# daniabib/ComfyUI_ProPainter_Nodes

Hardware: NVIDIA H100
Metric: inpainted frames/sec at 640x360, 80-frame subvideo (higher is better)
Workload: dtype f16

## Files before the change

### comfyui_propainter_nodes_b200/csrc/capi.cu

```cuda
#include <math.h>
#include <string.h>

#include <thread>
#include <vector>

#include "../../include/propainter_b200.h"
#include "engine.cuh"

struct DeviceGuard {
  int prev = -1;
  bool changed = false, ok = true;
  explicit DeviceGuard(int dev) {
    if (cudaGetDevice(&prev) != cudaSuccess) prev = -1;
    if (prev != dev) {
      ok = cudaSetDevice(dev) == cudaSuccess;
      changed = ok;
    }
  }
  ~DeviceGuard() {
    if (changed && prev >= 0) cudaSetDevice(prev);
  }
};

#define PP_HANDLE(h)                                     \
// ... 409 lines not shown
    a.n++; a.ms += ms; a.rows += r.rows; a.flops += r.flops; a.bytes += r.bytes;
  }
  size_t off = 0;
  buf[0] = 0;
  for (auto& kv : agg) {
    char line[512];
    int n = snprintf(line, sizeof(line), "%s\t%lld\t%.6f\t%.0f\t%.0f\t%.0f\n", kv.first.c_str(), kv.second.n,
                     kv.second.ms, kv.second.rows, kv.second.flops, kv.second.bytes);
    if (off + n + 1 > cap) { pp_set_error("pp_profile_dump: buffer too small"); return PP_ERR_ARG; }
    memcpy(buf + off, line, n + 1);
    off += n;
  }
  return PP_OK;
}

int pp_op_conv(pp_handle h, const char* name, const void* x_f16, int N, int H, int W, int stride, int pad, int dil,
               int replicate, int act, float slope, const void* residual_f16, void* out_f16, void* stream) {
  PP_HANDLE(h);
  const PPPackedConv* w = nullptr;
  PP_TRY(pp_get_conv(e, name, &w));
  PPConvCall c(e, name, N, H, W);
  c.in(static_cast<const __half*>(x_f16), w->cin_g * w->groups, 0, w->cin_g, w->groups > 1 ? w->cin_g : 0)
      .geom(stride, stride, pad, pad, dil, dil, replicate)
      .out(static_cast<__half*>(out_f16), w->cout_g * w->groups, 0, w->groups > 1 ? w->cout_g : 0)
      .act(act, slope);
  if (residual_f16 != nullptr) c.residual(static_cast<const __half*>(residual_f16), w->cout_g * w->groups, 0);
  return c.run(as_stream(stream));
}

int pp_op_corr_lookup(pp_handle h, const void* l0, const void* l1, const void* l2, const void* l3,
                      const float* coords, void* out_f16, long long nq, int h8, int w8, void* stream) {
  PP_HANDLE(h);
  e.launches++;
  return pp_k_corr_lookup(static_cast<const __half*>(l0), static_cast<const __half*>(l1),
                          static_cast<const __half*>(l2), static_cast<const __half*>(l3), coords,
                          static_cast<__half*>(out_f16), 328, nq, h8, w8, as_stream(stream));
}

int pp_op_conv_tf32(pp_handle h, const char* name, const float* x0, int x0_C, int x0_co, int x0_ch, const float* x1,
                    int x1_C, int x1_co, int x1_ch, int N, int H, int W, int sh, int sw, int ph, int pw, int dh, int dw,
                    int replicate, int epi, int act, float slope, float scale, int act2, const float* aux0, int aux0_C, int aux0_co, float* aux1,
// ... 117 lines not shown
```

### comfyui_propainter_nodes_b200/csrc/conv_epilogue.cuh

```cuda
#pragma once
#include "conv_igemm.cuh"
#include "wgmma_ops.cuh"

namespace ppconv {

template <int ACT, bool ACC = false, int N>
__device__ __forceinline__ void act16_t(float (&v)[N], float slope) {
#pragma unroll
  for (int i = 0; i < N; ++i) {
    if (ACT == PP_ACT_RELU) v[i] = fmaxf(v[i], 0.f);
    else if (ACT == PP_ACT_LRELU) v[i] = v[i] > 0.f ? v[i] : v[i] * slope;
    else if (ACT == PP_ACT_SIGMOID) v[i] = ppx::sigmoidf_(v[i]);
    else if (ACT == PP_ACT_TANH) v[i] = ACC ? ppx::tanh_acc(v[i]) : tanhf(v[i]);
    else if (ACT == PP_ACT_GELU) v[i] = ppx::gelu_erf(v[i]);
  }
}
template <bool ACC = false, int N>
__device__ __forceinline__ void act16(float (&v)[N], int act, float slope) {
  switch (act) {
    case PP_ACT_RELU: act16_t<PP_ACT_RELU, ACC>(v, slope); break;
    case PP_ACT_LRELU: act16_t<PP_ACT_LRELU, ACC>(v, slope); break;
    case PP_ACT_SIGMOID: act16_t<PP_ACT_SIGMOID, ACC>(v, slope); break;
    case PP_ACT_TANH: act16_t<PP_ACT_TANH, ACC>(v, slope); break;
    case PP_ACT_GELU: act16_t<PP_ACT_GELU, ACC>(v, slope); break;
// ... 232 lines not shown
#pragma unroll
    for (int i = 0; i < 16; i += 4) {
      const float4 v = *reinterpret_cast<const float4*>(src + i);
      acc[i] = v.x; acc[i + 1] = v.y; acc[i + 2] = v.z; acc[i + 3] = v.w;
    }
    conv_epilogue16_split(p, acc, mrow, g, ng0, p.vec_ok != 0);
  } else {
    uint32_t raw[16];
#pragma unroll
    for (int i = 0; i < 16; i += 4) {
      const float4 v = *reinterpret_cast<const float4*>(src + i);
      raw[i] = __float_as_uint(v.x); raw[i + 1] = __float_as_uint(v.y);
      raw[i + 2] = __float_as_uint(v.z); raw[i + 3] = __float_as_uint(v.w);
    }
    conv_epilogue16(p, raw, mrow, g, ng0, EPI >= 0 ? EPI : p.epi, p.vec_ok != 0);
  }
}

template <int V>
struct IntC { static constexpr int value = V; };
template <int MAX_N, class F>
__device__ __forceinline__ void with_tile_width(int bn, F&& f) {
  switch (bn) {
    case 16: f(IntC<16>{}); break;
    case 32: f(IntC<32>{}); break;
    case 48: f(IntC<48>{}); break;
    case 64: f(IntC<64>{}); break;
    case 80: f(IntC<80>{}); break;
    case 96: f(IntC<96>{}); break;
    case 112: f(IntC<112>{}); break;
// ... 22 lines not shown
```

### comfyui_propainter_nodes_b200/csrc/conv_halo.cu

```cuda
#include <cuda.h>
#include <stdlib.h>
#include <string.h>

#include <memory>

#include "conv_epilogue.cuh"
#include "conv_igemm.cuh"
#include "dcn_sample.cuh"

namespace {

constexpr int NUM_THREADS = 384;
constexpr int NUM_EPI_THREADS = 256;
constexpr int WARP_A = 8, WARP_B = 9;
constexpr int MAX_SA = 4, MAX_SB = 8;
constexpr int SMEM_BUDGET = 186 * 1024;

struct HaloParams {
  PPConvParams c;
  CUtensorMap tmap[PP_MAX_SEGS];
  int MT;
  int BW, BH;
  int tiles_x, tiles_y, n_tiles;
  int a_stage_bytes, b_stage_bytes, SA, SB;
// ... 16 lines not shown
  t.ty = r % h.tiles_y; r /= h.tiles_y;
  t.img = r % h.n_img;
  t.g = r / h.n_img;
  return t;
}

__host__ __device__ inline int halo_total_tiles(const HaloParams& h) {
  return h.n_tiles * h.tiles_x * h.tiles_y * h.n_img * h.c.groups;
}

struct Ring {
  int s;
  uint32_t ph;
};

struct HaloSmem {
  uint8_t* a;
  uint8_t* b;
  int SA, SB, a_stage_bytes, b_stage_bytes;
  uint64_t *a_full, *a_empty, *b_full, *b_empty;
  uint64_t* spare;
  float* acc_stg;
  int bytes;
};

__host__ __device__ inline HaloSmem halo_smem(uint8_t* base, int SA, int a_stage_bytes, int SB, int b_stage_bytes) {
  const int b_off = SA * a_stage_bytes, bar_off = b_off + SB * b_stage_bytes, acc_off = bar_off + 1024;
  HaloSmem m;
  m.SA = SA; m.SB = SB; m.a_stage_bytes = a_stage_bytes; m.b_stage_bytes = b_stage_bytes;
  m.a = base;
  m.b = base + b_off;
  m.a_full = reinterpret_cast<uint64_t*>(base + bar_off);
  m.a_empty = m.a_full + MAX_SA;
  m.b_full = m.a_empty + MAX_SA;
  m.b_empty = m.b_full + MAX_SB;
  m.spare = m.b_empty + MAX_SB;
  m.acc_stg = reinterpret_cast<float*>(base + acc_off);
  m.bytes = 1024 + acc_off + 2 * ppconv::STG_BYTES;
  return m;
}

__host__ __device__ constexpr int halo_max_tps(int bn) { return 128 / bn > 1 ? 128 / bn : 1; }

template <int BN, int MB, bool TF32>
__device__ __forceinline__ void halo_tap(float (&acc)[MB][BN / 2], uint64_t (&adesc)[MB], uint64_t& bdesc, uint32_t& accum,
                                         int& kx, int kw, uint32_t step_x, uint32_t step_row, uint32_t tap16) {
#pragma unroll
  for (int k = 0; k < 4; ++k)
#pragma unroll
    for (int b = 0; b < MB; ++b) {
      if constexpr (TF32) ppx::wgmma_tf32<BN>(acc[b], adesc[b] + 2 * k, bdesc + 2 * k, (accum | k) != 0 ? 1u : 0u);
      else ppx::wgmma_f16<BN>(acc[b], adesc[b] + 2 * k, bdesc + 2 * k, (accum | k) != 0 ? 1u : 0u);
    }
  accum = 1u;
// ... 9 lines not shown
                                               uint32_t& accum, int& kx, int kw, uint32_t step_x, uint32_t step_row,
                                               uint32_t tap16) {
  using namespace ppx;
  if constexpr (NT > 1) {
    if (tn < NT) {
      halo_tap_group<BN, MB, NT - 1, TF32>(tn, acc, adesc, bdesc, accum, kx, kw, step_x, step_row, tap16);
      return;
    }
  }
  wgmma_fence();
#pragma unroll
  for (int tt = 0; tt < NT; ++tt) halo_tap<BN, MB, TF32>(acc, adesc, bdesc, accum, kx, kw, step_x, step_row, tap16);
  wgmma_commit();
}

template <int BN, int MB, int NT, bool TF32 = false, bool PROG = false>
__device__ __forceinline__ void halo_tile(const HaloParams& h, int tile, const HaloSmem& m, Ring& ra, Ring& rb, float* stg,
                                          int wg, int t128) {
  using namespace ppx;
  const PPConvParams& p = h.c;
  const int taps = p.kh * p.kw;
  const TileCoord t = decode_tile(h, tile);
  const int n0 = t.n_idx * p.BN;
  const int bnt = min(p.BN, p.Cout_g_pad - n0);
  const uint32_t sbo = h.flat ? 1024u : (uint32_t)h.BW * 128;
  const uint32_t step_x = (uint32_t)p.dw * 8;
  const uint32_t step_row = (uint32_t)(p.dh * h.BW - (p.kw - 1) * p.dw) * 8;
  const uint32_t tap16 = (uint32_t)p.BN * 8;
  const int kw = p.kw;
  uint32_t aoff[MB];
#pragma unroll
  for (int b = 0; b < MB; ++b) aoff[b] = MB == 2 ? wg * h.sub_bytes + b * 8 * sbo : wg * 8 * sbo;
  float acc[MB][BN / 2];
// ... 6 lines not shown
    for (int b = 0; b < MB; ++b) adesc[b] = gmma_desc_sw128_kmajor(smem_u32(m.a + ra.s * m.a_stage_bytes) + aoff[b], sbo);
    int kx = 0;
    for (int tap0 = 0; tap0 < taps; tap0 += h.tps) {
      mbar_wait(&m.b_full[rb.s], rb.ph);
      const uint64_t bdesc = gmma_desc_sw128_kmajor(smem_u32(m.b + rb.s * m.b_stage_bytes));
      halo_tap_group<BN, MB, NT, TF32>(min(h.tps, taps - tap0), acc, adesc, bdesc, accum, kx, kw, step_x, step_row, tap16);
      wgmma_wait<1>();
      if (pend_b >= 0) mbar_arrive(&m.b_empty[pend_b]);
      if (pend_a >= 0) mbar_arrive(&m.a_empty[pend_a]);
      pend_b = rb.s;
      pend_a = tap0 + h.tps >= taps ? ra.s : -1;
      if (++rb.s == m.SB) { rb.s = 0; rb.ph ^= 1; }
    }
    if (++ra.s == m.SA) { ra.s = 0; ra.ph ^= 1; }
  }
  wgmma_wait<0>();
#pragma unroll
  for (int b = 0; b < MB; ++b) wgmma_fence_acc(acc[b]);
  if (pend_b >= 0) mbar_arrive(&m.b_empty[pend_b]);
  if (pend_a >= 0) mbar_arrive(&m.a_empty[pend_a]);

  const bool skip = (h.debug & 1) != 0;
#pragma unroll
  for (int b = 0; b < MB; ++b) {
    const int sub = MB == 2 ? wg : 0, rbase = MB == 2 ? 64 * b : 64 * wg;
    ppconv::drain_acc<BN>(acc[b], stg, t128, 4 + wg, [&](const float* src, int r64, int cc) {
      const int r = rbase + r64;
      bool mvalid;
      long long mrow;
      if (h.flat) {
        mrow = ((long long)t.tx * h.MT + sub) * 128 + r;
        mvalid = mrow < p.M_total;
      } else {
        const int oy = t.ty * 16 + (r >> 3), ox = t.tx * (8 * h.MT) + 8 * sub + (r & 7);
        mvalid = oy < p.OH && ox < p.OW;
        mrow = ((long long)t.img * p.OH + oy) * p.OW + ox;
      }
      if (!mvalid || skip || cc >= bnt || n0 + cc >= p.Cout_g) return;
      ppconv::epilogue_from_stage<TF32, PROG ? PP_EPI_STD : -1>(p, src, mrow, t.g, n0 + cc);
    });
  }
}

template <class F>
__device__ __forceinline__ void with_tile_shape(int mt, int bn, F&& f) {
  if (mt == 2) ppconv::with_tile_width<128>(bn, [&](auto n) { f(n, ppconv::IntC<2>{}); });
  else ppconv::with_tile_width<256>(bn, [&](auto n) { f(n, ppconv::IntC<1>{}); });
}

__device__ __forceinline__ void halo_smem_init_barriers(const HaloSmem& m) {
  using namespace ppx;
  for (int s = 0; s < m.SA; ++s) { mbar_init(&m.a_full[s], 1); mbar_init(&m.a_empty[s], NUM_EPI_THREADS); }
  for (int s = 0; s < m.SB; ++s) { mbar_init(&m.b_full[s], 1); mbar_init(&m.b_empty[s], NUM_EPI_THREADS); }
  mbar_fence_init();
}

__device__ __forceinline__ void halo_produce_patches(const HaloParams& h, const HaloSmem& m, Ring& r) {
  using namespace ppx;
  const PPConvParams& p = h.c;
  const int total_tiles = halo_total_tiles(h);
  const uint32_t bytes = (uint32_t)(h.BW * h.BH * 128);
  for (int tile = blockIdx.x; tile < total_tiles; tile += gridDim.x) {
// ... 39 lines not shown

template <bool TF32>
__device__ __forceinline__ void halo_body(const HaloParams& h) {
  using namespace ppx;
  const HaloSmem m = halo_smem(dyn_smem_1024(), h.SA, h.a_stage_bytes, h.SB, h.b_stage_bytes);
  const int tid = threadIdx.x, warp = tid >> 5;
  if (tid == 0) halo_smem_init_barriers(m);
  __syncthreads();
  asm volatile("griddepcontrol.wait;" ::: "memory");
  asm volatile("griddepcontrol.launch_dependents;" ::: "memory");

  if (warp < 8) setmaxnreg_inc<232>();
  else setmaxnreg_dec<40>();
  if (warp < 8) {
    const int wg = tid >> 7, t128 = tid & 127;
    float* stg = m.acc_stg + wg * (ppconv::STG_BYTES / 4);
    Ring ra = {0, 0}, rb = {0, 0};
    const int total_tiles = halo_total_tiles(h);
    with_tile_shape(h.MT, h.c.BN, [&](auto bn, auto mb) {
      constexpr int BN = decltype(bn)::value;
      for (int tile = blockIdx.x; tile < total_tiles; tile += gridDim.x)
        halo_tile<BN, decltype(mb)::value, halo_max_tps(BN), TF32>(h, tile, m, ra, rb, stg, wg, t128);
    });
  } else if (warp == WARP_A) {
    if (elect_one()) {
      Ring r = {0, 0};
      halo_produce_patches(h, m, r);
    }
  } else if (warp == WARP_B) {
    if (elect_one()) {
      Ring r = {0, 0};
      halo_produce_weights(h, m, r);
    }
  }
}

__global__ void __launch_bounds__(NUM_THREADS, 1) conv_halo_kernel(const __grid_constant__ HaloParams h) {
  halo_body<false>(h);
}

__global__ void __launch_bounds__(NUM_THREADS, 1) conv_halo_tf32_kernel(const __grid_constant__ HaloParams h) {
  halo_body<true>(h);
}

constexpr int PROG_MAX_LAYERS = 10;
enum { PROG_CONV = 0, PROG_DCN = 1 };

constexpr int PROG_WIDTHS[] = {32, 64, 224};

template <class F>
__device__ __forceinline__ void with_prog_width(int bn, F&& f) {
  static_assert(sizeof(PROG_WIDTHS) == 3 * sizeof(int), "with_prog_width: one case per PROG_WIDTHS entry");
  switch (bn) {
    case PROG_WIDTHS[0]: f(ppconv::IntC<PROG_WIDTHS[0]>{}); break;
    case PROG_WIDTHS[1]: f(ppconv::IntC<PROG_WIDTHS[1]>{}); break;
    case PROG_WIDTHS[2]: f(ppconv::IntC<PROG_WIDTHS[2]>{}); break;
    default: __trap();
  }
}

struct ProgParams {
  int n_layers;
  int SA, SB, a_stage_bytes, b_stage_bytes;
// ... 28 lines not shown

  const int tid = threadIdx.x, warp = tid >> 5;
  const unsigned int G = gridDim.x;
  if (tid == 0) {
    mbar_init(layer_go, 1);
    halo_smem_init_barriers(m);
  }
  __syncthreads();
  asm volatile("griddepcontrol.wait;" ::: "memory");
  asm volatile("griddepcontrol.launch_dependents;" ::: "memory");

  if (warp < 8) setmaxnreg_inc<232>();
  else setmaxnreg_dec<40>();
  if (warp < 8) {
    const int wg = tid >> 7, t128 = tid & 127;
    float* stg = m.acc_stg + wg * (ppconv::STG_BYTES / 4);
    Ring ra = {0, 0}, rb = {0, 0};
    for (int li = 0; li < P.n_layers; ++li) {
      mbar_wait(layer_go, (uint32_t)li & 1u);
      if (P.ts != nullptr && blockIdx.x == 0 && tid == 0) {
        unsigned long long now;
        asm volatile("mov.u64 %0, %%globaltimer;" : "=l"(now));
        P.ts[2 * li] = now;
      }
      if (P.kind[li] == PROG_DCN) {
        const PPDcnArgs& a = P.dcn[li];
        const unsigned per_img = (unsigned)(a.H * a.W * 144);
        const unsigned total = per_img * (unsigned)a.N;
        const unsigned stride = G * NUM_EPI_THREADS;
        for (unsigned idx = blockIdx.x * NUM_EPI_THREADS + tid; idx < total; idx += 4 * stride) {
#pragma unroll
          for (int u = 0; u < 4; ++u) {
            const unsigned i2 = idx + u * stride;
            if (i2 < total) {
              const unsigned n = i2 / per_img;
              if (a.C == 128) dcn_sample_item<8, true>(a, i2 - n * per_img, (int)n);
              else dcn_sample_item<16, true>(a, i2 - n * per_img, (int)n);
            }
          }
        }
      } else {
        const HaloParams& h = P.layer[li];
        const int total_tiles = halo_total_tiles(h);
        with_prog_width(h.c.BN, [&](auto bn) {
          constexpr int BN = decltype(bn)::value;
          for (int tile = blockIdx.x; tile < total_tiles; tile += G)
            halo_tile<BN, 1, halo_max_tps(BN), false, true>(h, tile, m, ra, rb, stg, wg, t128);
        });
      }
      fence_proxy_async_global();
      asm volatile("bar.sync 1, %0;" ::"n"(NUM_EPI_THREADS) : "memory");
      if (tid == 0) {
        __threadfence();
        atomicAdd(P.counter, 1u);
        if (P.ts != nullptr && blockIdx.x == 0) {
          unsigned long long now;
          asm volatile("mov.u64 %0, %%globaltimer;" : "=l"(now));
          P.ts[2 * li + 1] = now;
        }
      }
    }
  } else if (warp == WARP_A) {
// ... 74 lines not shown
  int mt = count(2, bn) < num_sms ? 1 : 2;
  while (count(mt, bn) < num_sms && bn >= 64 && bn % 32 == 0) bn /= 2;
  if (one_wave) {
    mt = 1;
    long long best_cols = -1, best_waves = 0;
    for (const int b : PROG_WIDTHS) {
      const long long waves = (count(1, b) + num_sms - 1) / num_sms;
      if (best_cols < 0 || waves * b < best_cols || (waves * b == best_cols && waves < best_waves)) {
        best_cols = waves * b;
        best_waves = waves;
        bn = b;
      }
    }
  }
  p.BN = bn;
  h.MT = mt;
  h.flat = flat ? 1 : 0;
  h.n_img = n_img;
  h.BW = flat ? 128 * mt : 8 * mt + (p.kw - 1) * p.dw;
  h.BH = flat ? 1 : 16 + (p.kh - 1) * p.dh;
  h.sub_bytes = flat ? 128 * 128 : 8 * 128;
  h.tiles_x = tiles_x(mt);
  h.tiles_y = tiles_y;
  h.n_tiles = pp_ceil_div(p.Cout_g_pad, bn);
  h.chunks = pp_ceil_div(p.Cin, 64);
  h.a_stage_bytes = pp_ceil_div(h.BW * h.BH * 128, 1024) * 1024;
  h.tps = min(halo_max_tps(bn), p.kh * p.kw);
  h.b_stage_bytes = h.tps * bn * 128;
  int sa = 0, sb = 0;
  PP_REQUIRE(halo_stages(SMEM_BUDGET, h.a_stage_bytes, h.b_stage_bytes, sa, sb),
// ... 38 lines not shown
  return PP_OK;
}

void pp_prog_abort() {
  delete g_recorder;
  g_recorder = nullptr;
}

int pp_prog_record_conv(const PPConvParams& p) {
  PPProgRecorder* r = g_recorder;
  PP_REQUIRE(r != nullptr, "conv program: not recording");
  PP_REQUIRE(r->prog.n_layers < PROG_MAX_LAYERS, "conv program: more than %d layers", PROG_MAX_LAYERS);
  PP_REQUIRE(pp_conv_halo_eligible(p), "conv program: layer is not a stride-1 TMA halo-kernel convolution");
  PP_REQUIRE(!p.split, "conv program: split-tf32 layers are not supported");
  PP_REQUIRE(p.epi == PP_EPI_STD, "conv program: only the plain epilogue (bias, activations, residual) is compiled in");
  const int li = r->prog.n_layers;
  PP_TRY(halo_configure(p, r->prog.layer[li], true));
  const HaloParams& h = r->prog.layer[li];
  PP_REQUIRE(h.MT == 1 && (h.c.BN == PROG_WIDTHS[0] || h.c.BN == PROG_WIDTHS[1] || h.c.BN == PROG_WIDTHS[2]),
             "conv program: layer tile %d x %d columns is not instantiated", h.MT, h.c.BN);
  r->prog.kind[li] = PROG_CONV;
  r->prog.n_layers++;
  r->n_conv++;
  return PP_OK;
}

int pp_prog_record_dcn(const PPDcnArgs& a) {
  PPProgRecorder* r = g_recorder;
  PP_REQUIRE(r != nullptr, "conv program: not recording");
  PP_REQUIRE(r->prog.n_layers < PROG_MAX_LAYERS, "conv program: more than %d layers", PROG_MAX_LAYERS);
// ... 59 lines not shown
```

### comfyui_propainter_nodes_b200/engine.py

```python
from __future__ import annotations

import ctypes
import math
import os
from typing import Dict, Tuple

import torch

from . import weights as Wspec

_LIB = None
_PKG_DIR = os.path.dirname(os.path.abspath(__file__))
LIB_PATH = os.environ.get("PP_LIB_PATH") or os.path.join(_PKG_DIR, "libpropainter_b200.so")

MAX_BN = 256
ACT_NONE, ACT_RELU, ACT_LRELU, ACT_SIGMOID, ACT_TANH, ACT_GELU = range(6)

_VP, _I, _F, _LL, _SZ, _CP = (ctypes.c_void_p, ctypes.c_int, ctypes.c_float, ctypes.c_longlong, ctypes.c_size_t,
                              ctypes.c_char_p)
_SIGNATURES = {
    "pp_last_error": (_CP, []),
    "pp_version": (_CP, []),
    "pp_create": (_I, [_I, _VP, _SZ, ctypes.POINTER(_VP)]),
    "pp_destroy": (_I, [_VP]),
# ... 16 lines not shown
    "pp_gen_begin": (_I, [_VP, _VP, _VP, _VP, _VP, _VP, _I, _I, _I, _VP]),
    "pp_gen_begin_subset": (_I, [_VP, _VP, _VP, _VP, _VP, _VP, _I, _I, _I, ctypes.c_char_p, _VP]),
    "pp_gen_window": (_I, [_VP, ctypes.POINTER(_I), _I, _I, _VP, _VP]),
    "pp_gen_run": (_I, [_VP, ctypes.POINTER(_I), ctypes.POINTER(_I), ctypes.POINTER(_I), _I, _VP, _VP]),
    "pp_gen_end": (_I, [_VP]),
    "pp_composite": (_I, [_VP, _VP, _VP, _VP, _VP, _VP, _VP, _I, _I, _I, _I, _VP]),
    "pp_preprocess": (_I, [_VP, _VP, _VP, _I, _I, _I, _I, _I, _I, _VP, _VP, _VP, _VP, _VP]),
    "pp_preprocess_resize": (_I, [_VP, _VP, _VP, _I, _I, _I, _I, _I, _I, _I, _I, _VP, _VP, _VP, _VP, _VP]),
    "pp_preprocess_u8": (_I, [_VP, _VP, _VP, _I, _I, _I, _I, _I, _I, _I, _I, _VP, _VP, _VP, _VP, _VP]),
    "pp_host_quantize_u8": (_I, [_VP, _VP, _LL, _I]),
    "pp_postprocess": (_I, [_VP, _VP, _VP, _LL, _VP]),
    "pp_launch_count": (_LL, [_VP]),
    "pp_workspace_peak": (_SZ, [_VP]),
    "pp_profile_enable": (_I, [_VP, _I]),
    "pp_profile_dump": (_I, [_VP, ctypes.c_char_p, _SZ]),
    "pp_op_conv": (_I, [_VP, _CP, _VP, _I, _I, _I, _I, _I, _I, _I, _I, _F, _VP, _VP, _VP]),
    "pp_op_corr_lookup": (_I, [_VP, _VP, _VP, _VP, _VP, _VP, _VP, _LL, _I, _I, _VP]),
    "pp_op_conv_tf32": (_I, [_VP, _CP, _VP, _I, _I, _I, _VP, _I, _I, _I, _I, _I, _I, _I, _I, _I, _I, _I, _I, _I, _I, _I,
                             _F, _F, _I, _VP, _I, _I, _VP, _I, _I, _VP, _I, _I, _I, _VP]),
    "pp_op_dcn_sample_f32": (_I, [_VP, _VP, _I, _VP, _I, _VP, _I, _I, _I, _F, _VP, _VP]),
    "pp_op_upsample2x_f32": (_I, [_VP, _VP, _VP, _I, _I, _I, _I, _VP]),
    "pp_op_instnorm": (_I, [_VP, _VP, _VP, _VP, _I, _I, _I, _I, _I, _VP]),
    "pp_op_corr_pyramid": (_I, [_VP, _VP, _VP, _I, _I, _I, _I, _VP, _VP, _VP, _VP, _VP]),
    "pp_op_corr_lookup_f32": (_I, [_VP, _VP, _VP, _VP, _VP, _VP, _VP, _LL, _I, _I, _VP]),
    "pp_op_convex_upsample": (_I, [_VP, _VP, _VP, _VP, _I, _I, _I, _I, _VP]),
    "pp_op_imgprop_step": (_I, [_VP, _VP, _VP, _VP, _VP, _VP, _I, _I, _VP]),
    "pp_op_imgprop_step_f32": (_I, [_VP, _VP, _VP, _VP, _VP, _VP, _I, _I, _VP]),
    "pp_op_attention": (_I, [_VP, _VP, _VP, _VP, _VP, _I, _I, _I, _I, _I, _VP]),
}


# ... 558 lines not shown
    def workspace_peak(self) -> int:
        return int(self.lib.pp_workspace_peak(self.h))

    def profile_enable(self, on: bool):
        self._check(self.lib.pp_profile_enable(self.h, int(on)))

    def profile_dump(self):
        buf = ctypes.create_string_buffer(1 << 20)
        self._check(self.lib.pp_profile_dump(self.h, buf, len(buf)))
        out = {}
        for line in buf.value.decode().splitlines():
            name, n, ms, rows, flops, nbytes = line.split("\t")
            out[name] = dict(count=int(n), ms=float(ms), rows=float(rows), flops=float(flops), bytes=float(nbytes))
        return out

    def op_conv(self, name, x_nhwc, stride=1, pad=0, dil=1, replicate=False, act=ACT_NONE, slope=0.0, residual=None):
        m = self.conv_meta[name]
        N, H, W, _ = x_nhwc.shape
        kh, kw = m["kh"], m["kw"]
        OH = (H + 2 * pad - dil * (kh - 1) - 1) // stride + 1
        OW = (W + 2 * pad - dil * (kw - 1) - 1) // stride + 1
        out = torch.empty(N, OH, OW, m["cout_g"] * m["groups"], device=self.device, dtype=torch.float16)
        self._check(self.lib.pp_op_conv(self.h, name.encode(), _ptr(x_nhwc), N, H, W, stride, pad, dil, int(replicate),
                                        act, float(slope), _ptr(residual), _ptr(out), self._stream()))
        return out

    def op_corr_lookup(self, levels, coords, h8, w8):
        nq = coords.shape[0]
        out = torch.empty(nq, 328, device=self.device, dtype=torch.float16)
        self._check(self.lib.pp_op_corr_lookup(self.h, *[_ptr(l) for l in levels], _ptr(coords), _ptr(out), nq, h8, w8,
                                               self._stream()))
        return out

    EPI_STD, EPI_GRU_ZR, EPI_GRU_H = range(3)

    def op_conv_tf32(self, name, inputs, out, out_co=0, stride=(1, 1), pad=(0, 0), act=ACT_NONE, slope=0.0, scale=1.0,
                     act2=ACT_NONE, residual=None, gru_zr=None, gru_h=None, out_fp32=False, dilation=(1, 1),
                     replicate=False):
        N, H, W = inputs[0][0].shape[:3]
# ... 77 lines not shown
```

### include/propainter_b200.h

```cpp
#ifndef PROPAINTER_B200_H
#define PROPAINTER_B200_H

#include <stddef.h>
#include <stdint.h>

#ifdef __cplusplus
extern "C" {
#endif

#if defined(__GNUC__)
#define PP_API __attribute__((visibility("default")))
#else
#define PP_API
#endif

typedef struct PPEngine* pp_handle;

PP_API const char* pp_last_error(void);
PP_API const char* pp_version(void);

PP_API int pp_create(int device, void* workspace, size_t workspace_bytes, pp_handle* out);
PP_API int pp_destroy(pp_handle h);
PP_API int pp_set_workspace(pp_handle h, void* workspace, size_t workspace_bytes);

// ... 46 lines not shown
PP_API int pp_preprocess_resize(pp_handle h, const float* image, const float* mask, int mask_frames, int T, int H, int W,
                                int out_h, int out_w, int flow_mask_dilates, int mask_dilates, uint8_t* orig_u8,
                                float* frames, float* flow_masks, float* masks_dilated, void* stream);
PP_API int pp_preprocess_u8(pp_handle h, const uint8_t* image_u8, const uint8_t* mask_u8, int mask_frames, int T, int H,
                            int W, int out_h, int out_w, int flow_mask_dilates, int mask_dilates, uint8_t* orig_u8,
                            float* frames, float* flow_masks, float* masks_dilated, void* stream);
PP_API int pp_host_quantize_u8(const float* src, uint8_t* dst, long long n, int threads);
PP_API int pp_postprocess(pp_handle h, const uint8_t* comp_u8, float* image_out, long long n, void* stream);

PP_API long long pp_launch_count(pp_handle h);
PP_API size_t pp_workspace_peak(pp_handle h);

PP_API int pp_profile_enable(pp_handle h, int on);
PP_API int pp_profile_dump(pp_handle h, char* buf, size_t cap);

PP_API int pp_op_conv(pp_handle h, const char* name, const void* x_f16, int N, int H, int W, int stride, int pad, int dil,
               int replicate, int act, float slope, const void* residual_f16, void* out_f16, void* stream);
PP_API int pp_op_corr_lookup(pp_handle h, const void* l0, const void* l1, const void* l2, const void* l3,
                      const float* coords, void* out_f16, long long nq, int h8, int w8, void* stream);
PP_API int pp_op_conv_tf32(pp_handle h, const char* name, const float* x0, int x0_C, int x0_co, int x0_ch, const float* x1,
                           int x1_C, int x1_co, int x1_ch, int N, int H, int W, int sh, int sw, int ph, int pw, int dh,
                           int dw, int replicate, int epi, int act, float slope, float scale, int act2, const float* aux0, int aux0_C, int aux0_co,
                           float* aux1, int aux1_C, int aux1_co, float* out, int out_C, int out_co, int out_fp32,
                           void* stream);
PP_API int pp_op_dcn_sample_f32(pp_handle h, const float* x0, int C0, const float* x1, int C1, const float* offs, int N,
                                int H, int W, float max_mag, float* cols, void* stream);
PP_API int pp_op_upsample2x_f32(pp_handle h, const float* src, float* dst, int N, int H, int W, int C, void* stream);
PP_API int pp_op_instnorm(pp_handle h, const void* x, const void* residual, void* out, int N, int HW, int C, int relu,
                          int fp32, void* stream);
PP_API int pp_op_corr_pyramid(pp_handle h, const void* fmap1, const void* fmap2, int pairs, int h8, int w8, int fp32,
                              void* l0, void* l1, void* l2, void* l3, void* stream);
PP_API int pp_op_corr_lookup_f32(pp_handle h, const float* l0, const float* l1, const float* l2, const float* l3,
// ... 15 lines not shown
```

Baseline: 168.9.

## Prefetch epilogue operands during MMA and specialize halo conv epilogues

The f16 halo-conv epilogue now loads residual and GRU aux tensors into registers before waiting on the wgmma accumulators. It also stages bias in shared memory and drains accumulators through a double-buffered staging area with one barrier per chunk. GRU and activation epilogue variants are specialized at compile time. This is meant to hide global-load latency and barrier cost in the epilogue, at the price of more shared memory, registers and template instantiations. The conv op API is also widened to expose these epilogues.

Measured after the change: 172.6 (median of 6 runs). +2.2%, better.

```diff
diff --git a/comfyui_propainter_nodes_b200/csrc/capi.cu b/comfyui_propainter_nodes_b200/csrc/capi.cu
--- a/comfyui_propainter_nodes_b200/csrc/capi.cu
+++ b/comfyui_propainter_nodes_b200/csrc/capi.cu
@@ -447,17 +447,29 @@
   return PP_OK;
 }
 
-int pp_op_conv(pp_handle h, const char* name, const void* x_f16, int N, int H, int W, int stride, int pad, int dil,
-               int replicate, int act, float slope, const void* residual_f16, void* out_f16, void* stream) {
-  PP_HANDLE(h);
+int pp_op_conv(pp_handle h, const char* name, const void* x0, int x0_cs, int x0_co, int x0_ch, const void* x1, int x1_cs,
+               int x1_co, int x1_ch, int N, int H, int W, int sh, int sw, int ph, int pw, int dh, int dw, int replicate,
+               int epi, int act, float slope, float scale, int act2, const void* aux0, int aux0_cs, int aux0_co, void* aux1,
+               int aux1_cs, int aux1_co, void* out, int out_cs, int out_co, void* stream) {
+  PP_HANDLE(h);
+  PP_REQUIRE(name && x0 && out, "pp_op_conv: null pointer");
+  PP_REQUIRE(epi == PP_EPI_STD || (aux0 && aux1), "pp_op_conv: the GRU epilogues need aux0 and aux1");
   const PPPackedConv* w = nullptr;
   PP_TRY(pp_get_conv(e, name, &w));
+  const auto* a0 = static_cast<const __half*>(aux0);
+  auto* a1 = static_cast<__half*>(aux1);
   PPConvCall c(e, name, N, H, W);
-  c.in(static_cast<const __half*>(x_f16), w->cin_g * w->groups, 0, w->cin_g, w->groups > 1 ? w->cin_g : 0)
-      .geom(stride, stride, pad, pad, dil, dil, replicate)
-      .out(static_cast<__half*>(out_f16), w->cout_g * w->groups, 0, w->groups > 1 ? w->cout_g : 0)
-      .act(act, slope);
-  if (residual_f16 != nullptr) c.residual(static_cast<const __half*>(residual_f16), w->cout_g * w->groups, 0);
+  c.in(static_cast<const __half*>(x0), x0_cs, x0_co, x0_ch, w->groups > 1 ? w->cin_g : 0);
+  if (x1 != nullptr) c.in(static_cast<const __half*>(x1), x1_cs, x1_co, x1_ch);
+  c.geom(sh, sw, ph, pw, dh, dw, replicate).out(static_cast<__half*>(out), out_cs, out_co, w->groups > 1 ? w->cout_g : 0);
+  if (epi == PP_EPI_GRU_ZR) {
+    c.gru_zr(a0, aux0_cs, aux0_co, a1, aux1_cs, aux1_co);
+  } else if (epi == PP_EPI_GRU_H) {
+    c.gru_h(a0, aux0_cs, aux0_co, a1, aux1_cs, aux1_co);
+  } else {
+    c.act(act, slope, scale, act2);
+    if (a0 != nullptr) c.residual(a0, aux0_cs, aux0_co);
+  }
   return c.run(as_stream(stream));
 }
 
diff --git a/comfyui_propainter_nodes_b200/csrc/conv_epilogue.cuh b/comfyui_propainter_nodes_b200/csrc/conv_epilogue.cuh
--- a/comfyui_propainter_nodes_b200/csrc/conv_epilogue.cuh
+++ b/comfyui_propainter_nodes_b200/csrc/conv_epilogue.cuh
@@ -270,6 +270,216 @@
       raw[i + 2] = __float_as_uint(v.z); raw[i + 3] = __float_as_uint(v.w);
     }
     conv_epilogue16(p, raw, mrow, g, ng0, EPI >= 0 ? EPI : p.epi, p.vec_ok != 0);
+  }
+}
+
+
+struct Aux16 {
+  uint4 lo, hi;
+};
+struct AuxPair {
+  Aux16 a0, a1;
+};
+
+__device__ __forceinline__ uint32_t pack_halves(__half a, __half b) {
+  return (uint32_t)__half_as_ushort(a) | ((uint32_t)__half_as_ushort(b) << 16);
+}
+
+__device__ __forceinline__ void aux_load16(Aux16& a, const __half* src, int nvalid, bool vec) {
+  if (vec && nvalid == 16) {
+    a.lo = reinterpret_cast<const uint4*>(src)[0];
+    a.hi = reinterpret_cast<const uint4*>(src)[1];
+  } else {
+    const __half z = __ushort_as_half(0);
+    uint32_t w[8];
+#pragma unroll
+    for (int k = 0; k < 8; ++k) w[k] = pack_halves(2 * k < nvalid ? src[2 * k] : z, 2 * k + 1 < nvalid ? src[2 * k + 1] : z);
+    a.lo = make_uint4(w[0], w[1], w[2], w[3]);
+    a.hi = make_uint4(w[4], w[5], w[6], w[7]);
+  }
+}
+
+__device__ __forceinline__ void aux_unpack16(const Aux16& a, float (&r)[16]) {
+  const uint32_t w[8] = {a.lo.x, a.lo.y, a.lo.z, a.lo.w, a.hi.x, a.hi.y, a.hi.z, a.hi.w};
+#pragma unroll
+  for (int k = 0; k < 8; ++k) {
+    r[2 * k] = __half2float(__ushort_as_half((unsigned short)(w[k] & 0xFFFFu)));
+    r[2 * k + 1] = __half2float(__ushort_as_half((unsigned short)(w[k] >> 16)));
+  }
+}
+
+__device__ __forceinline__ void store16_pieces(__half* dst, int nvalid, bool vec, const float (&v)[16]) {
+  if (!vec) {
+    store16(dst, nvalid, false, v);
+    return;
+  }
+  uint32_t w[8];
+#pragma unroll
+  for (int k = 0; k < 8; ++k) {
+    const __half2 h = __floats2half2_rn(v[2 * k], v[2 * k + 1]);
+    w[k] = pack_halves(__low2half(h), __high2half(h));
+  }
+  if (nvalid == 16) {
+    reinterpret_cast<uint4*>(dst)[0] = make_uint4(w[0], w[1], w[2], w[3]);
+    reinterpret_cast<uint4*>(dst)[1] = make_uint4(w[4], w[5], w[6], w[7]);
+    return;
+  }
+  const bool p8 = (nvalid & 8) != 0;
+  if (p8) reinterpret_cast<uint4*>(dst)[0] = make_uint4(w[0], w[1], w[2], w[3]);
+  if (nvalid & 4) {
+    const int o = nvalid & 8;
+    *reinterpret_cast<uint2*>(dst + o) = p8 ? make_uint2(w[4], w[5]) : make_uint2(w[0], w[1]);
+  }
+  if (nvalid & 2) {
+    const int o = nvalid & 12;
+    uint32_t x = w[0];
+#pragma unroll
+    for (int k = 1; k < 7; ++k)
+      if (2 * k == o) x = w[k];
+    *reinterpret_cast<uint32_t*>(dst + o) = x;
+  }
+  if (nvalid & 1) {
+    const int o = nvalid & 14;
+    uint32_t x = w[0];
+#pragma unroll
+    for (int k = 1; k < 8; ++k)
+      if (2 * k == o) x = w[k];
+    dst[o] = __ushort_as_half((unsigned short)(x & 0xFFFFu));
+  }
+}
+
+template <int EPI>
+__device__ __forceinline__ void epi_prefetch(const PPConvParams& p, AuxPair& a, long long mrow, int ng0, bool vec) {
+  const int nvalid = min(16, p.Cout_g - ng0);
+  if constexpr (EPI == PP_EPI_STD) {
+    if (p.aux0 != nullptr) aux_load16(a.a0, p.aux0 + mrow * p.aux0_cstride + p.aux0_coff + ng0, nvalid, vec);
+  } else if constexpr (EPI == PP_EPI_GRU_ZR) {
+    const int half_c = p.Cout_g >> 1;
+    if (ng0 >= half_c) aux_load16(a.a0, p.aux0 + mrow * p.aux0_cstride + p.aux0_coff + (ng0 - half_c), nvalid, vec);
+  } else {
+    aux_load16(a.a0, p.aux0 + mrow * p.aux0_cstride + p.aux0_coff + ng0, nvalid, vec);
+    aux_load16(a.a1, p.aux1 + mrow * p.aux1_cstride + p.aux1_coff + ng0, nvalid, vec);
+  }
+}
+
+template <int EPI, int ACT1 = -1>
+__device__ __forceinline__ void conv_epilogue16_pf(const PPConvParams& p, float (&v)[16], const float* bs, const AuxPair& a,
+                                                   long long mrow, int g, int ng0, bool vec) {
+  const int nvalid = min(16, p.Cout_g - ng0);
+  if (bs != nullptr) {
+#pragma unroll
+    for (int i = 0; i < 4; ++i) {
+      const float4 b4 = reinterpret_cast<const float4*>(bs)[i];
+      v[4 * i] += b4.x; v[4 * i + 1] += b4.y; v[4 * i + 2] += b4.z; v[4 * i + 3] += b4.w;
+    }
+  }
+  if constexpr (EPI == PP_EPI_STD) {
+    if constexpr (ACT1 >= 0) act16_t<ACT1>(v, p.slope);
+    else act16(v, p.act1, p.slope);
+    if (p.scale != 1.f) {
+#pragma unroll
+      for (int i = 0; i < 16; ++i) v[i] *= p.scale;
+    }
+    if (p.aux0 != nullptr) {
+      float r[16];
+      aux_unpack16(a.a0, r);
+#pragma unroll
+      for (int i = 0; i < 16; ++i) v[i] += r[i];
+    }
+    if constexpr (ACT1 < 0) act16(v, p.act2, p.slope);
+    const long long o = mrow * p.out_cstride + p.out_coff + (long long)g * p.out_gstep + ng0;
+    if (p.out_fp32) {
+      float* dst = reinterpret_cast<float*>(p.out) + o;
+      if (vec && nvalid == 16) {
+#pragma unroll
+        for (int i = 0; i < 4; ++i)
+          reinterpret_cast<float4*>(dst)[i] = make_float4(v[4 * i], v[4 * i + 1], v[4 * i + 2], v[4 * i + 3]);
+      } else {
+#pragma unroll
+        for (int i = 0; i < 16; ++i)
+          if (i < nvalid) dst[i] = v[i];
+      }
+    } else {
+      store16_pieces(reinterpret_cast<__half*>(p.out) + o, nvalid, vec, v);
+    }
+  } else if constexpr (EPI == PP_EPI_GRU_ZR) {
+    const int half_c = p.Cout_g >> 1;
+    act16_t<PP_ACT_SIGMOID>(v, 0.f);
+    if (ng0 < half_c) {
+      store16_pieces(reinterpret_cast<__half*>(p.out) + mrow * p.out_cstride + p.out_coff + ng0, nvalid, vec, v);
+    } else {
+      const int c = ng0 - half_c;
+      float h[16];
+      aux_unpack16(a.a0, h);
+#pragma unroll
+      for (int i = 0; i < 16; ++i) v[i] *= h[i];
+      store16_pieces(p.out2 + mrow * p.out2_cstride + p.out2_coff + c, nvalid, vec, v);
+    }
+  } else {
+    float h[16], z[16];
+    aux_unpack16(a.a0, h);
+    aux_unpack16(a.a1, z);
+    act16_t<PP_ACT_TANH>(v, 0.f);
+#pragma unroll
+    for (int i = 0; i < 16; ++i) v[i] = (1.f - z[i]) * h[i] + z[i] * v[i];
+    store16_pieces(reinterpret_cast<__half*>(p.out) + mrow * p.out_cstride + p.out_coff + ng0, nvalid, vec, v);
+  }
+}
+
+constexpr int STG2_FLOATS = 64 * 32;
+constexpr int STG2_BYTES = 2 * STG2_FLOATS * 4;
+__device__ __forceinline__ int stg2_at(int row, int col) {
+  const int q = row & 3;
+  return row * 32 + (((col >> 2) ^ ((q << 1) | (q >> 1))) << 2) + (col & 3);
+}
+
+template <int N, int MB, class Aux, class Pre, class Emit>
+__device__ __forceinline__ void drain_acc_1bar(const float (&acc)[MB][N / 2], float* stg, uint32_t& flip, int bar_id,
+                                               const Aux& first, Pre&& pre, Emit&& emit) {
+  constexpr int NCH = (N + 31) / 32;
+  uint32_t tid;
+  asm volatile("mov.u32 %0, %%tid.x;" : "=r"(tid));
+  const int t128 = (int)(tid & 127);
+  const int wrow = 16 * (t128 >> 5) + ((t128 & 31) >> 2), wcol = 2 * (t128 & 3);
+  const int rrow = t128 >> 1, rcol = 16 * (t128 & 1);
+  Aux cur = first;
+#pragma unroll 1
+  for (int r = 0; r < MB * NCH; ++r) {
+    const int b = r / NCH, c0 = (r - b * NCH) * 32;
+    float* s = stg + (flip & 1) * STG2_FLOATS;
+    flip ^= 1;
+#pragma unroll
+    for (int bb = 0; bb < MB; ++bb)
+#pragma unroll
+      for (int cc = 0; cc < N; cc += 32) {
+        if (bb == b && cc == c0) {
+#pragma unroll
+          for (int j = 0; j < 4; ++j) {
+            if (cc + 8 * j < N) {
+              const int i = (cc / 8 + j) * 4;
+              *reinterpret_cast<float2*>(s + stg2_at(wrow, 8 * j + wcol)) = make_float2(acc[bb][i], acc[bb][i + 1]);
+              *reinterpret_cast<float2*>(s + stg2_at(wrow + 8, 8 * j + wcol)) = make_float2(acc[bb][i + 2], acc[bb][i + 3]);
+            }
+          }
+        }
+      }
+    Aux nxt = cur;
+    if (r + 1 < MB * NCH) {
+      const int b1 = (r + 1) / NCH;
+      pre(nxt, b1, rrow, (r + 1 - b1 * NCH) * 32 + rcol);
+    }
+    ppx::named_bar(bar_id, 128);
+    const int c = c0 + rcol;
+    if (c < N) {
+      float v[16];
+#pragma unroll
+      for (int i = 0; i < 4; ++i) {
+        const float4 f = *reinterpret_cast<const float4*>(s + stg2_at(rrow, rcol + 4 * i));
+        v[4 * i] = f.x; v[4 * i + 1] = f.y; v[4 * i + 2] = f.z; v[4 * i + 3] = f.w;
+      }
+      emit(v, b, rrow, c, cur);
+    }
+    cur = nxt;
   }
 }
 
diff --git a/comfyui_propainter_nodes_b200/csrc/conv_halo.cu b/comfyui_propainter_nodes_b200/csrc/conv_halo.cu
--- a/comfyui_propainter_nodes_b200/csrc/conv_halo.cu
+++ b/comfyui_propainter_nodes_b200/csrc/conv_halo.cu
@@ -54,6 +54,8 @@
   uint32_t ph;
 };
 
+constexpr int STG_WG_BYTES = ppconv::STG2_BYTES > ppconv::STG_BYTES ? ppconv::STG2_BYTES : ppconv::STG_BYTES;
+constexpr int BIAS_WG_FLOATS = 256;
 struct HaloSmem {
   uint8_t* a;
   uint8_t* b;
@@ -66,6 +68,7 @@
 
 __host__ __device__ inline HaloSmem halo_smem(uint8_t* base, int SA, int a_stage_bytes, int SB, int b_stage_bytes) {
   const int b_off = SA * a_stage_bytes, bar_off = b_off + SB * b_stage_bytes, acc_off = bar_off + 1024;
+  const int bias_off = acc_off + 2 * STG_WG_BYTES;
   HaloSmem m;
   m.SA = SA; m.SB = SB; m.a_stage_bytes = a_stage_bytes; m.b_stage_bytes = b_stage_bytes;
   m.a = base;
@@ -76,8 +79,12 @@
   m.b_empty = m.b_full + MAX_SB;
   m.spare = m.b_empty + MAX_SB;
   m.acc_stg = reinterpret_cast<float*>(base + acc_off);
-  m.bytes = 1024 + acc_off + 2 * ppconv::STG_BYTES;
+  m.bytes = 1024 + bias_off + 2 * BIAS_WG_FLOATS * 4;
   return m;
+}
+
+__device__ __forceinline__ float* halo_bias_smem(const HaloSmem& m, int wg) {
+  return m.acc_stg + 2 * STG_WG_BYTES / 4 + wg * BIAS_WG_FLOATS;
 }
 
 __host__ __device__ constexpr int halo_max_tps(int bn) { return 128 / bn > 1 ? 128 / bn : 1; }
@@ -117,9 +124,9 @@
   wgmma_commit();
 }
 
-template <int BN, int MB, int NT, bool TF32 = false, bool PROG = false>
+template <int BN, int MB, int NT, bool TF32, int EPI, int ACT1 = -1>
 __device__ __forceinline__ void halo_tile(const HaloParams& h, int tile, const HaloSmem& m, Ring& ra, Ring& rb, float* stg,
-                                          int wg, int t128) {
+                                          float* bs, uint32_t& flip, int wg, int t128) {
   using namespace ppx;
   const PPConvParams& p = h.c;
   const int taps = p.kh * p.kw;
@@ -156,31 +163,70 @@
     }
     if (++ra.s == m.SA) { ra.s = 0; ra.ph ^= 1; }
   }
-  wgmma_wait<0>();
-#pragma unroll
-  for (int b = 0; b < MB; ++b) wgmma_fence_acc(acc[b]);
-  if (pend_b >= 0) mbar_arrive(&m.b_empty[pend_b]);
-  if (pend_a >= 0) mbar_arrive(&m.a_empty[pend_a]);
 
   const bool skip = (h.debug & 1) != 0;
-#pragma unroll
-  for (int b = 0; b < MB; ++b) {
-    const int sub = MB == 2 ? wg : 0, rbase = MB == 2 ? 64 * b : 64 * wg;
-    ppconv::drain_acc<BN>(acc[b], stg, t128, 4 + wg, [&](const float* src, int r64, int cc) {
-      const int r = rbase + r64;
-      bool mvalid;
+  auto live = [&](int b, int r64, int cc, long long& mrow) {
+    const int sub = MB == 2 ? wg : 0;
+    const int r = (MB == 2 ? 64 * b : 64 * wg) + r64;
+    bool mvalid;
+    if (h.flat) {
+      mrow = ((long long)t.tx * h.MT + sub) * 128 + r;
+      mvalid = mrow < p.M_total;
+    } else {
+      const int oy = t.ty * 16 + (r >> 3), ox = t.tx * (8 * h.MT) + 8 * sub + (r & 7);
+      mvalid = oy < p.OH && ox < p.OW;
+      mrow = ((long long)t.img * p.OH + oy) * p.OW + ox;
+    }
+    return mvalid && !skip && cc < bnt && n0 + cc < p.Cout_g;
+  };
+  if constexpr (TF32) {
+    wgmma_wait<0>();
+#pragma unroll
+    for (int b = 0; b < MB; ++b) wgmma_fence_acc(acc[b]);
+    if (pend_b >= 0) mbar_arrive(&m.b_empty[pend_b]);
+    if (pend_a >= 0) mbar_arrive(&m.a_empty[pend_a]);
+#pragma unroll
+    for (int b = 0; b < MB; ++b) {
+      ppconv::drain_acc<BN>(acc[b], stg, t128, 4 + wg, [&](const float* src, int r64, int cc) {
+        long long mrow;
+        if (live(b, r64, cc, mrow)) ppconv::epilogue_from_stage<true>(p, src, mrow, t.g, n0 + cc);
+      });
+    }
+  } else {
+    const bool vec = p.vec_ok != 0;
+    constexpr int NB = (BN + 127) / 128;
+    float bias_r[NB];
+    const bool has_bias = p.bias != nullptr;
+#pragma unroll
+    for (int k = 0; k < NB; ++k) {
+      const int c = t128 + 128 * k;
+      bias_r[k] = has_bias && c < BN && n0 + c < p.Cout_g ? __ldg(p.bias + t.g * p.Cout_g + n0 + c) : 0.f;
+    }
+    ppconv::AuxPair first = {};
+    {
       long long mrow;
-      if (h.flat) {
-        mrow = ((long long)t.tx * h.MT + sub) * 128 + r;
-        mvalid = mrow < p.M_total;
-      } else {
-        const int oy = t.ty * 16 + (r >> 3), ox = t.tx * (8 * h.MT) + 8 * sub + (r & 7);
-        mvalid = oy < p.OH && ox < p.OW;
-        mrow = ((long long)t.img * p.OH + oy) * p.OW + ox;
-      }
-      if (!mvalid || skip || cc >= bnt || n0 + cc >= p.Cout_g) return;
-      ppconv::epilogue_from_stage<TF32, PROG ? PP_EPI_STD : -1>(p, src, mrow, t.g, n0 + cc);
-    });
+      if (live(0, t128 >> 1, 16 * (t128 & 1), mrow)) ppconv::epi_prefetch<EPI>(p, first, mrow, n0 + 16 * (t128 & 1), vec);
+    }
+    wgmma_wait<0>();
+#pragma unroll
+    for (int b = 0; b < MB; ++b) wgmma_fence_acc(acc[b]);
+    if (pend_b >= 0) mbar_arrive(&m.b_empty[pend_b]);
+    if (pend_a >= 0) mbar_arrive(&m.a_empty[pend_a]);
+    named_bar(4 + wg, 128);
+#pragma unroll
+    for (int k = 0; k < NB; ++k)
+      if (t128 + 128 * k < BN) bs[t128 + 128 * k] = bias_r[k];
+    ppconv::drain_acc_1bar<BN, MB>(
+        acc, stg, flip, 4 + wg, first,
+        [&](ppconv::AuxPair& a, int b, int r64, int cc) {
+          long long mrow;
+          if (live(b, r64, cc, mrow)) ppconv::epi_prefetch<EPI>(p, a, mrow, n0 + cc, vec);
+        },
+        [&](float (&v)[16], int b, int r64, int cc, const ppconv::AuxPair& a) {
+          long long mrow;
+          if (live(b, r64, cc, mrow))
+            ppconv::conv_epilogue16_pf<EPI, ACT1>(p, v, has_bias ? bs + cc : nullptr, a, mrow, t.g, n0 + cc, vec);
+        });
   }
 }
 
@@ -188,6 +234,33 @@
 __device__ __forceinline__ void with_tile_shape(int mt, int bn, F&& f) {
   if (mt == 2) ppconv::with_tile_width<128>(bn, [&](auto n) { f(n, ppconv::IntC<2>{}); });
   else ppconv::with_tile_width<256>(bn, [&](auto n) { f(n, ppconv::IntC<1>{}); });
+}
+
+constexpr int GRU_WIDTHS[] = {32, 64, 128};
+
+template <class F>
+__device__ __forceinline__ void with_tile_case(int mt, int bn, int epi, F&& f) {
+  using ppconv::IntC;
+  static_assert(sizeof(GRU_WIDTHS) == 3 * sizeof(int), "with_tile_case: one case per GRU_WIDTHS entry");
+  if (epi == PP_EPI_STD) {
+    with_tile_shape(mt, bn, [&](auto n, auto m) { f(n, m, IntC<PP_EPI_STD>{}); });
+    return;
+  }
+  auto gru = [&](auto e) {
+    auto widths = [&](auto m) {
+      switch (bn) {
+        case GRU_WIDTHS[0]: f(IntC<GRU_WIDTHS[0]>{}, m, e); break;
+        case GRU_WIDTHS[1]: f(IntC<GRU_WIDTHS[1]>{}, m, e); break;
+        case GRU_WIDTHS[2]: f(IntC<GRU_WIDTHS[2]>{}, m, e); break;
+        default: __trap();
+      }
+    };
+    if (mt == 2) widths(IntC<2>{});
+    else widths(IntC<1>{});
+  };
+  if (epi == PP_EPI_GRU_ZR) gru(IntC<PP_EPI_GRU_ZR>{});
+  else if (epi == PP_EPI_GRU_H) gru(IntC<PP_EPI_GRU_H>{});
+  else __trap();
 }
 
 __device__ __forceinline__ void halo_smem_init_barriers(const HaloSmem& m) {
@@ -257,14 +330,25 @@
   else setmaxnreg_dec<40>();
   if (warp < 8) {
     const int wg = tid >> 7, t128 = tid & 127;
-    float* stg = m.acc_stg + wg * (ppconv::STG_BYTES / 4);
+    float* stg = m.acc_stg + wg * (STG_WG_BYTES / 4);
+    float* bs = halo_bias_smem(m, wg);
+    uint32_t flip = 0;
     Ring ra = {0, 0}, rb = {0, 0};
     const int total_tiles = halo_total_tiles(h);
-    with_tile_shape(h.MT, h.c.BN, [&](auto bn, auto mb) {
-      constexpr int BN = decltype(bn)::value;
-      for (int tile = blockIdx.x; tile < total_tiles; tile += gridDim.x)
-        halo_tile<BN, decltype(mb)::value, halo_max_tps(BN), TF32>(h, tile, m, ra, rb, stg, wg, t128);
-    });
+    if constexpr (TF32) {
+      with_tile_shape(h.MT, h.c.BN, [&](auto bn, auto mb) {
+        constexpr int BN = decltype(bn)::value;
+        for (int tile = blockIdx.x; tile < total_tiles; tile += gridDim.x)
+          halo_tile<BN, decltype(mb)::value, halo_max_tps(BN), true, -1>(h, tile, m, ra, rb, stg, bs, flip, wg, t128);
+      });
+    } else {
+      with_tile_case(h.MT, h.c.BN, h.c.epi, [&](auto bn, auto mb, auto epi) {
+        constexpr int BN = decltype(bn)::value;
+        for (int tile = blockIdx.x; tile < total_tiles; tile += gridDim.x)
+          halo_tile<BN, decltype(mb)::value, halo_max_tps(BN), false, decltype(epi)::value>(h, tile, m, ra, rb, stg, bs,
+                                                                                            flip, wg, t128);
+      });
+    }
   } else if (warp == WARP_A) {
     if (elect_one()) {
       Ring r = {0, 0};
@@ -290,6 +374,7 @@
 enum { PROG_CONV = 0, PROG_DCN = 1 };
 
 constexpr int PROG_WIDTHS[] = {32, 64, 224};
+constexpr int PROG_ACTS[] = {PP_ACT_NONE, PP_ACT_LRELU};
 
 template <class F>
 __device__ __forceinline__ void with_prog_width(int bn, F&& f) {
@@ -348,7 +433,7 @@
   else setmaxnreg_dec<40>();
   if (warp < 8) {
     const int wg = tid >> 7, t128 = tid & 127;
-    float* stg = m.acc_stg + wg * (ppconv::STG_BYTES / 4);
+    float* stg = m.acc_stg + wg * (STG_WG_BYTES / 4);
     Ring ra = {0, 0}, rb = {0, 0};
     for (int li = 0; li < P.n_layers; ++li) {
       mbar_wait(layer_go, (uint32_t)li & 1u);
@@ -376,10 +461,18 @@
       } else {
         const HaloParams& h = P.layer[li];
         const int total_tiles = halo_total_tiles(h);
+        float* bs = halo_bias_smem(m, wg);
+        uint32_t flip = 0;
         with_prog_width(h.c.BN, [&](auto bn) {
           constexpr int BN = decltype(bn)::value;
-          for (int tile = blockIdx.x; tile < total_tiles; tile += G)
-            halo_tile<BN, 1, halo_max_tps(BN), false, true>(h, tile, m, ra, rb, stg, wg, t128);
+          auto tiles = [&](auto act) {
+            for (int tile = blockIdx.x; tile < total_tiles; tile += G)
+              halo_tile<BN, 1, halo_max_tps(BN), false, PP_EPI_STD, decltype(act)::value>(h, tile, m, ra, rb, stg, bs, flip,
+                                                                                         wg, t128);
+          };
+          constexpr int ACT_A = PROG_ACTS[0], ACT_B = PROG_ACTS[1];
+          if (h.c.act1 == ACT_B) tiles(ppconv::IntC<ACT_B>{});
+          else tiles(ppconv::IntC<ACT_A>{});
         });
       }
       fence_proxy_async_global();
@@ -484,6 +577,8 @@
     }
   }
   p.BN = bn;
+  PP_REQUIRE(p.split || p.epi == PP_EPI_STD || bn == GRU_WIDTHS[0] || bn == GRU_WIDTHS[1] || bn == GRU_WIDTHS[2],
+             "conv_halo: the GRU epilogues are not compiled for %d-column tiles (%d output channels)", bn, p.Cout_g);
   h.MT = mt;
   h.flat = flat ? 1 : 0;
   h.n_img = n_img;
@@ -552,6 +647,8 @@
   PP_REQUIRE(pp_conv_halo_eligible(p), "conv program: layer is not a stride-1 TMA halo-kernel convolution");
   PP_REQUIRE(!p.split, "conv program: split-tf32 layers are not supported");
   PP_REQUIRE(p.epi == PP_EPI_STD, "conv program: only the plain epilogue (bias, activations, residual) is compiled in");
+  PP_REQUIRE((p.act1 == PROG_ACTS[0] || p.act1 == PROG_ACTS[1]) && p.act2 == PP_ACT_NONE,
+             "conv program: activation %d / %d is not compiled in", p.act1, p.act2);
   const int li = r->prog.n_layers;
   PP_TRY(halo_configure(p, r->prog.layer[li], true));
   const HaloParams& h = r->prog.layer[li];
diff --git a/comfyui_propainter_nodes_b200/engine.py b/comfyui_propainter_nodes_b200/engine.py
--- a/comfyui_propainter_nodes_b200/engine.py
+++ b/comfyui_propainter_nodes_b200/engine.py
@@ -54,7 +54,8 @@
     "pp_workspace_peak": (_SZ, [_VP]),
     "pp_profile_enable": (_I, [_VP, _I]),
     "pp_profile_dump": (_I, [_VP, ctypes.c_char_p, _SZ]),
-    "pp_op_conv": (_I, [_VP, _CP, _VP, _I, _I, _I, _I, _I, _I, _I, _I, _F, _VP, _VP, _VP]),
+    "pp_op_conv": (_I, [_VP, _CP, _VP, _I, _I, _I, _VP, _I, _I, _I, _I, _I, _I, _I, _I, _I, _I, _I, _I, _I, _I, _I, _F,
+                        _F, _I, _VP, _I, _I, _VP, _I, _I, _VP, _I, _I, _VP]),
     "pp_op_corr_lookup": (_I, [_VP, _VP, _VP, _VP, _VP, _VP, _VP, _LL, _I, _I, _VP]),
     "pp_op_conv_tf32": (_I, [_VP, _CP, _VP, _I, _I, _I, _VP, _I, _I, _I, _I, _I, _I, _I, _I, _I, _I, _I, _I, _I, _I, _I,
                              _F, _F, _I, _VP, _I, _I, _VP, _I, _I, _VP, _I, _I, _I, _VP]),
@@ -643,15 +644,30 @@
             out[name] = dict(count=int(n), ms=float(ms), rows=float(rows), flops=float(flops), bytes=float(nbytes))
         return out
 
-    def op_conv(self, name, x_nhwc, stride=1, pad=0, dil=1, replicate=False, act=ACT_NONE, slope=0.0, residual=None):
+    def op_conv(self, name, x_nhwc, stride=1, pad=0, dil=1, replicate=False, act=ACT_NONE, slope=0.0, residual=None, *,
+                x1=None, out=None, out_co=0, scale=1.0, act2=ACT_NONE, gru_zr=None, gru_h=None):
         m = self.conv_meta[name]
-        N, H, W, _ = x_nhwc.shape
+        x0, c0, n0 = (x_nhwc, 0, m["cin_g"]) if torch.is_tensor(x_nhwc) else x_nhwc
+        x1, c1, n1 = (None, 0, 0) if x1 is None else x1
+        N, H, W = x0.shape[:3]
         kh, kw = m["kh"], m["kw"]
-        OH = (H + 2 * pad - dil * (kh - 1) - 1) // stride + 1
-        OW = (W + 2 * pad - dil * (kw - 1) - 1) // stride + 1
-        out = torch.empty(N, OH, OW, m["cout_g"] * m["groups"], device=self.device, dtype=torch.float16)
-        self._check(self.lib.pp_op_conv(self.h, name.encode(), _ptr(x_nhwc), N, H, W, stride, pad, dil, int(replicate),
-                                        act, float(slope), _ptr(residual), _ptr(out), self._stream()))
+        ph, pw = pad if isinstance(pad, tuple) else (pad, pad)
+        OH = (H + 2 * ph - dil * (kh - 1) - 1) // stride + 1
+        OW = (W + 2 * pw - dil * (kw - 1) - 1) // stride + 1
+        if out is None:
+            out = torch.empty(N, OH, OW, m["cout_g"] * m["groups"], device=self.device, dtype=torch.float16)
+        epi, a0, a0_co, a1, a1_co = self.EPI_STD, None, 0, None, 0
+        if residual is not None:
+            a0, a0_co = (residual, 0) if torch.is_tensor(residual) else residual
+        if gru_zr is not None:
+            epi, (a0, a0_co, a1, a1_co) = self.EPI_GRU_ZR, gru_zr
+        if gru_h is not None:
+            epi, (a0, a0_co, a1, a1_co) = self.EPI_GRU_H, gru_h
+        cs = lambda t: 0 if t is None else t.shape[-1]
+        self._check(self.lib.pp_op_conv(
+            self.h, name.encode(), _ptr(x0), cs(x0), c0, n0, _ptr(x1), cs(x1), c1, n1, N, H, W, stride, stride, ph, pw,
+            dil, dil, int(replicate), epi, act, float(slope), float(scale), act2, _ptr(a0), cs(a0), a0_co, _ptr(a1), cs(a1),
+            a1_co, _ptr(out), cs(out), out_co, self._stream()))
         return out
 
     def op_corr_lookup(self, levels, coords, h8, w8):
diff --git a/include/propainter_b200.h b/include/propainter_b200.h
--- a/include/propainter_b200.h
+++ b/include/propainter_b200.h
@@ -84,8 +84,10 @@
 PP_API int pp_profile_enable(pp_handle h, int on);
 PP_API int pp_profile_dump(pp_handle h, char* buf, size_t cap);
 
-PP_API int pp_op_conv(pp_handle h, const char* name, const void* x_f16, int N, int H, int W, int stride, int pad, int dil,
-               int replicate, int act, float slope, const void* residual_f16, void* out_f16, void* stream);
+PP_API int pp_op_conv(pp_handle h, const char* name, const void* x0, int x0_cs, int x0_co, int x0_ch, const void* x1,
+                      int x1_cs, int x1_co, int x1_ch, int N, int H, int W, int sh, int sw, int ph, int pw, int dh, int dw,
+                      int replicate, int epi, int act, float slope, float scale, int act2, const void* aux0, int aux0_cs,
+                      int aux0_co, void* aux1, int aux1_cs, int aux1_co, void* out, int out_cs, int out_co, void* stream);
 PP_API int pp_op_corr_lookup(pp_handle h, const void* l0, const void* l1, const void* l2, const void* l3,
                       const float* coords, void* out_f16, long long nq, int h8, int w8, void* stream);
 PP_API int pp_op_conv_tf32(pp_handle h, const char* name, const float* x0, int x0_C, int x0_co, int x0_ch, const float* x1,
```
